# PRiME-project/PRiMEStereoMatch

Measured on AMD Instinct MI355X. Metric: cost-volume voxels/s (CVC+CVF+WTA), higher is better.
Workload: dtype f32; 1 GPU; synthetic 1920x1080 pair, D=256, float32 (BASELINE configs[3]); W=1920, H=1080, D=256, parallelism=1 GPU, kernel_variant=0, lr_check_on_gpu=False, batch=1, ranks=1, same_device=False, frames_in_flight=1

## Files before the change

include/primesm_hip.h:

```cpp
#ifndef PRIMESM_HIP_H
#define PRIMESM_HIP_H

#include <stddef.h>
#include <stdint.h>

#ifdef __cplusplus
extern "C" {
#endif

#define PSM_ABI_VERSION 1

typedef struct psm_ctx psm_ctx;

enum { PSM_F32 = 0, PSM_U8 = 1 };
enum { PSM_IMG_U8 = 0, PSM_IMG_F32 = 1 };
enum { PSM_LEFT = 0, PSM_RIGHT = 1 };
enum { PSM_STAGE_CVC = 0, PSM_STAGE_CVF = 1, PSM_STAGE_DISPSEL = 2, PSM_STAGE_PP = 3,
       PSM_STAGE_COUNT = 4 };
enum { PSM_K_PREP = 0, PSM_K_CVC = 1, PSM_K_GUIDE = 2, PSM_K_CVF_A = 3, PSM_K_CVF_B = 4,
       PSM_K_WTA = 5, PSM_K_MERGE = 6, PSM_K_BOX = 7, PSM_K_LRC = 8, PSM_K_CVF_F = 9, PSM_K_FGF = 10, PSM_K_WMF = 11,
       PSM_K_JWMF = 12, PSM_K_COUNT = 13 };
enum {
    PSM_OPT_ASYNC = 0,
    PSM_OPT_KERNEL_VARIANT = 1,
    PSM_OPT_PROFILE = 2,
    PSM_OPT_SEG_ROWS = 3,
    PSM_OPT_WAVES = 4,
    PSM_OPT_FLAGS = 5,
    PSM_OPT_GRAPH = 6,
    PSM_OPT_GATHER_STAGED = 7,
    PSM_OPT_FRAMES_IN_FLIGHT = 8
};

enum psm_flag {
    PSM_FLAG_MATERIALISE_COSTS = 128,
    PSM_FLAG_FGF_STORE = 4096,
    PSM_FLAG_STORE_FILTERED = 8192,
    PSM_FLAG_TWO_PHASE_ON = 1048576,
    PSM_FLAG_TWO_PHASE_OFF = 2097152,
    PSM_FLAG_WMF_DATAFLOW = 4194304,
    PSM_FLAG_WMF_TWO_SWEEPS = 8388608,
    PSM_FLAG_WMF_NO_CACHE = 16777216,
    PSM_FLAG_F32_TOL = 33554432,
    PSM_FLAG_FMA_SOLVE = 67108864,
    PSM_FLAGS_ALL = 128 | 4096 | 8192 | 1048576 | 2097152 | 4194304 | 8388608 | 16777216 | 33554432 | 67108864
};

int psm_device_count(void);

int psm_create(psm_ctx **out, int width, int height, int max_disp, int dtype, int device);

int psm_create_shard(psm_ctx **out, int width, int height, int max_disp, int d_begin, int d_end,
                     int dtype, int device);
int psm_create_shard_strided(psm_ctx **out, int width, int height, int max_disp, int d_first, int d_step,
                             int dtype, int device);

void psm_destroy(psm_ctx *ctx);

const char *psm_last_error(const psm_ctx *ctx);

int psm_set_option(psm_ctx *ctx, int option, int value);
int psm_set_stream(psm_ctx *ctx, void *hip_stream);
int psm_synchronize(psm_ctx *ctx);
int psm_release_scratch(psm_ctx *ctx);

int psm_upload_pair(psm_ctx *ctx, const void *l, const void *r, int channels, size_t stride_bytes,
                    int depth);

int psm_cost_construct(psm_ctx *ctx);

int psm_cost_filter(psm_ctx *ctx);

int psm_cost_filter_side(psm_ctx *ctx, int side);

int psm_cost_filter_fgf(psm_ctx *ctx, int subsample_rate);

int psm_disp_select(psm_ctx *ctx, uint8_t *lmap, uint8_t *rmap, size_t stride);

int psm_disp_select_partial(psm_ctx *ctx, void *dev_keys);
int psm_disp_select_partial_side(psm_ctx *ctx, int side, void *dev_keys_side);
int psm_set_key_buffer(psm_ctx *ctx, void *dev_keys);
int psm_partial_keys(psm_ctx *ctx, void **dev_keys, size_t *bytes);
int psm_disp_merge(psm_ctx *ctx, const void *dev_keys_all, int nranks, uint8_t *lmap,
                   uint8_t *rmap, size_t stride);
// ... 108 lines not shown
```

primestereomatch_amd/capi.py:

```python
from __future__ import annotations

import ctypes as C
import os

_HERE = os.path.dirname(os.path.abspath(__file__))
LIB_PATH = os.path.join(_HERE, "lib", "libprimesm_hip.so")

PSM_F32, PSM_U8 = 0, 1
PSM_IMG_U8, PSM_IMG_F32 = 0, 1
PSM_LEFT, PSM_RIGHT = 0, 1
PSM_STAGE_CVC, PSM_STAGE_CVF, PSM_STAGE_DISPSEL, PSM_STAGE_PP = 0, 1, 2, 3
(PSM_K_PREP, PSM_K_CVC, PSM_K_GUIDE, PSM_K_CVF_A, PSM_K_CVF_B, PSM_K_WTA, PSM_K_MERGE, PSM_K_BOX,
 PSM_K_LRC, PSM_K_CVF_F, PSM_K_FGF, PSM_K_WMF, PSM_K_JWMF) = range(13)
(PSM_OPT_ASYNC, PSM_OPT_KERNEL_VARIANT, PSM_OPT_PROFILE, PSM_OPT_SEG_ROWS, PSM_OPT_WAVES, PSM_OPT_FLAGS, PSM_OPT_GRAPH,
 PSM_OPT_GATHER_STAGED, PSM_OPT_FRAMES_IN_FLIGHT) = range(9)
PSM_FLAG_MATERIALISE_COSTS, PSM_FLAG_FGF_STORE, PSM_FLAG_STORE_FILTERED = 128, 4096, 8192
PSM_FLAG_TWO_PHASE_ON, PSM_FLAG_TWO_PHASE_OFF = 1048576, 2097152
PSM_FLAG_WMF_DATAFLOW, PSM_FLAG_WMF_TWO_SWEEPS, PSM_FLAG_WMF_NO_CACHE = 4194304, 8388608, 16777216
PSM_FLAG_F32_TOL = 33554432
PSM_FLAG_FMA_SOLVE = 67108864
PSM_SCORE_GIF, PSM_SCORE_SGM, PSM_SCORE_SGM_INT = 0, 1, 2
PSM_MASK_NONE, PSM_MASK_NONOCC, PSM_MASK_DISC = 0, 1, 2
PSM_SCORE_FLAT = 1


class Score(C.Structure):
    _fields_ = [("min_val", C.c_int32), ("max_val", C.c_int32), ("pixels", C.c_uint32), ("bad", C.c_uint32),
                ("err_sum", C.c_uint64), ("unit", C.c_int32), ("flags", C.c_uint32)]

    def as_dict(self):
        d = {name: int(getattr(self, name)) for name, _ in self._fields_}
        d["bp_percent"] = 100.0 * d["bad"] / d["pixels"]
        d["avg_err"] = (d["err_sum"] / d["pixels"]) / d["unit"] if d["unit"] else 0.0
        return d


_vp, _i, _sz = C.c_void_p, C.c_int, C.c_size_t
_pi, _pd = C.POINTER(C.c_int), C.POINTER(C.c_double)
SYMBOLS = [
    ("psm_device_count", _i, []),
    ("psm_create", _i, [C.POINTER(_vp), _i, _i, _i, _i, _i]),
    ("psm_create_shard", _i, [C.POINTER(_vp), _i, _i, _i, _i, _i, _i, _i]),
    ("psm_create_shard_strided", _i, [C.POINTER(_vp), _i, _i, _i, _i, _i, _i, _i]),
    ("psm_destroy", None, [_vp]),
    ("psm_last_error", C.c_char_p, [_vp]),
    ("psm_set_option", _i, [_vp, _i, _i]),
    ("psm_set_stream", _i, [_vp, _vp]),
    ("psm_synchronize", _i, [_vp]),
    ("psm_release_scratch", _i, [_vp]),
    ("psm_upload_pair", _i, [_vp, _vp, _vp, _i, _sz, _i]),
    ("psm_upload_pair_async", _i, [_vp, _vp, _vp, _i, _sz, _i]),
    ("psm_cost_construct", _i, [_vp]),
    ("psm_cost_filter", _i, [_vp]),
    ("psm_cost_filter_side", _i, [_vp, _i]),
    ("psm_cost_filter_fgf", _i, [_vp, _i]),
    ("psm_disp_select", _i, [_vp, _vp, _vp, _sz]),
    ("psm_disp_select_partial_side", _i, [_vp, _i, _vp]),
    ("psm_disp_select_partial", _i, [_vp, _vp]),
    ("psm_set_key_buffer", _i, [_vp, _vp]),
    ("psm_partial_keys", _i, [_vp, C.POINTER(_vp), C.POINTER(_sz)]),
    ("psm_disp_merge", _i, [_vp, _vp, _i, _vp, _vp, _sz]),
    ("psm_disp_merge_ctx", _i, [_vp, C.POINTER(_vp), _i, _vp, _vp, _sz]),
    ("psm_compute_batch", _i, [C.POINTER(_vp), _i]),
    ("psm_share_streams", _i, [C.POINTER(_vp), _i]),
    ("psm_download_maps", _i, [_vp, _vp, _vp, _sz]),
    ("psm_download_maps_async", _i, [_vp]),
    ("psm_download_maps_wait", _i, [_vp, _vp, _vp, _sz]),
    ("psm_lr_check", _i, [_vp, _vp, _vp, _sz]),
# ... 96 lines not shown
```

primestereomatch_amd/csrc/psm_api_core.cpp:

```cpp
#include "psm_ctx.h"

#include <chrono>
#include <cstdarg>
#include <cstdio>
#include <cstring>

using namespace psm;

namespace {
std::string g_create_error;
}

namespace psm {

double now_us()
{
    using namespace std::chrono;
    return duration_cast<duration<double, std::micro>>(steady_clock::now().time_since_epoch()).count();
}

int fail(psm_ctx *c, const char *fmt, ...)
{
    char buf[512];
    va_list ap;
// ... 296 lines not shown
    delete ctx;
}

const char *psm_last_error(const psm_ctx *ctx) { return ctx ? ctx->err.c_str() : g_create_error.c_str(); }

int psm_get_info(const psm_ctx *c, int *width, int *height, int *max_disp, int *d_begin, int *d_end, int *dtype, int *device)
{
    if (!c) return 1;
    if (width) *width = c->W;
    if (height) *height = c->H;
    if (max_disp) *max_disp = c->D;
    if (d_begin) *d_begin = c->d0;
    if (d_end) *d_end = c->d1;
    if (dtype) *dtype = c->dtype;
    if (device) *device = c->device;
    return 0;
}

int psm_set_option(psm_ctx *c, int option, int value)
{
    if (!c) return 1;
    switch (option) {
    case PSM_OPT_ASYNC: c->opt_async = value != 0; return 0;
    case PSM_OPT_KERNEL_VARIANT:
        if (value != 0 && value != 1) return fail(c, "psm_set_option: kernel variant %d unknown", value);
        c->opt_variant = value; return 0;
    case PSM_OPT_PROFILE:
        if (value < 0 || value > 2) return fail(c, "psm_set_option: profile mode %d not in {0,1,2}", value);
        c->opt_profile = value; return 0;
    case PSM_OPT_SEG_ROWS:
        if (value < 0) return fail(c, "psm_set_option: seg_rows %d < 0", value);
        c->march.seg_rows = value; return 0;
    case PSM_OPT_WAVES:
        if (value != 1 && value != 2 && value != 4 && value != 8) return fail(c, "psm_set_option: waves %d not in {1,2,4,8}", value);
        c->march.waves = value; return 0;
    case PSM_OPT_FLAGS:
        if (value & ~PSM_FLAGS_ALL) return fail(c, "psm_set_option: unknown flag bits 0x%x", value & ~PSM_FLAGS_ALL);
        if (c->dtype == PSM_U8) value &= ~(PSM_FLAG_FMA_SOLVE | PSM_FLAG_F32_TOL);
        if ((value & PSM_FLAG_F32_TOL) && (value & PSM_FLAG_FMA_SOLVE))
            return fail(c, "psm_set_option: PSM_FLAG_F32_TOL and PSM_FLAG_FMA_SOLVE exclude each other (one arithmetic variant at a time)");
        if ((value ^ c->march.flags) & PSM_FLAG_FMA_SOLVE) c->guid_rows = Rows{};
        c->march.flags = value; return 0;
    case PSM_OPT_GRAPH:
#ifdef PSM_EXPERIMENTS
        c->opt_graph = value != 0; return 0;
#else
        if (value != 0) return fail(c, "psm_set_option: PSM_OPT_GRAPH is not part of the product library (hipGraph replay of a batch measured slower than its plain launches)");
        return 0;
#endif
    case PSM_OPT_GATHER_STAGED: c->opt_gather_staged = value != 0; return 0;
    case PSM_OPT_FRAMES_IN_FLIGHT:
        if (value < 1 || value > 64) return fail(c, "psm_set_option: frames in flight %d not in [1, 64]", value);
        c->march.inflight = value; return 0;
    default: return fail(c, "psm_set_option: unknown option %d", option);
    }
}

int psm_set_stream(psm_ctx *c, void *hip_stream)
{
    if (!c) return 1;
    if (bind(c)) return 1;
    if (c->shared) return fail(c, "psm_set_stream: the context shares its streams with a batch (psm_share_streams)");
    PSM_HIP(c, hipStreamSynchronize(c->stream));
    c->stream = hip_stream ? (hipStream_t)hip_stream : c->own_stream;
    return 0;
}

int psm_synchronize(psm_ctx *c)
{
    if (!c) return 1;
    if (bind(c)) return 1;
    PSM_HIP(c, hipStreamSynchronize(c->stream));
    if (c->copy_stream) PSM_HIP(c, hipStreamSynchronize(c->copy_stream));
    if (c->down_stream && c->down_stream != c->copy_stream) PSM_HIP(c, hipStreamSynchronize(c->down_stream));
    return 0;
}

int psm_release_scratch(psm_ctx *c)
{
    if (!c) return 1;
    if (psm_synchronize(c)) return 1;
    (void)hipFree(c->wm_wts); c->wm_wts = nullptr; c->wm_wts_n = 0;
    (void)hipFree(c->wm_par); c->wm_par = nullptr;
    (void)hipFree(c->wm); c->wm = nullptr;
    (void)hipFree(c->gf_scratch); c->gf_scratch = nullptr; c->gf_scratch_bytes = 0;
    (void)hipFree(c->gather); c->gather = nullptr; c->gather_ranks = 0;
    (void)hipFree(c->fvol); c->fvol = nullptr;
    rectify_free(c, false);
    sgm_free(c);
    score_free(c, false);
    for (int k = 0; k < 2; ++k)
        if (c->xfer_pin[k]) { (void)hipHostFree(c->xfer_pin[k]); c->xfer_pin[k] = nullptr; c->xfer_pin_bytes[k] = 0; }
    (void)hipGetLastError();
    return 0;
}

int psm_share_streams(psm_ctx *const *ctxs, int n)
{
    if (!ctxs || n < 1 || !ctxs[0]) return fail(nullptr, "psm_share_streams: bad arguments");
    psm_ctx *c0 = ctxs[0];
    for (int i = 0; i < n; ++i) {
        if (!ctxs[i] || ctxs[i]->device != c0->device) return fail(c0, "psm_share_streams: context %d is NULL or on another device", i);
        if (ctxs[i]->shared) return fail(c0, "psm_share_streams: context %d already shares streams", i);
        for (int j = 0; j < i; ++j)
            if (ctxs[j] == ctxs[i]) return fail(c0, "psm_share_streams: context %d appears twice", i);
        if (ctxs[i]->stream != ctxs[i]->own_stream) return fail(c0, "psm_share_streams: context %d runs on a caller's stream (psm_set_stream)", i);
// ... 238 lines not shown
```

primestereomatch_amd/csrc/psm_kernels.h:

```cpp
#pragma once
#include <hip/hip_runtime.h>
#include <stdint.h>
#include "psm_live.h"

namespace psm {

struct Guidance {
    float4 *g1;
    float4 *g2;
    float4 *g3;
    float2 *g4;
};

struct March {
    int seg_rows;
    int waves;
    int flags;
    int dstep = 1;
    int inflight = 1;
    int ybeg = 0, yend = 0;
    int y0(int H) const { (void)H; return yend > ybeg ? ybeg : 0; }
    int y1(int H) const { return yend > ybeg ? yend : H; }
    int rows(int H) const { return y1(H) - y0(H); }
};

struct PcPair {
    const void *raw[2];
    Guidance g[2];
    uint8_t *p4[2];
    void *scratch;
    long long *keys;
    uint8_t *maps;
};
struct PcPairs {
    const PcPair *tab;
    int n;
    PcPair one;
};
void launch_prep_batch(hipStream_t s, const PcPair *tab, int npairs, size_t pitch, int depth_f32, int W, int H, bool u8_planes);
void launch_merge_batch(hipStream_t s, const PcPair *tab, int npairs, int W, int H);

void launch_copy_bytes(hipStream_t s, void *dst, const void *src, size_t bytes);
void launch_range_f32(hipStream_t s, const float *p, size_t n, unsigned *out);
void launch_prep(hipStream_t s, const void *src, size_t pitch, int depth_f32, int W, int H, float4 *g1, const void *src1 = nullptr,
                 float4 *g11 = nullptr);
void launch_guidance(hipStream_t s, const PcPairs &P, int W, int H, int ybeg, int yend, bool fma, int src = 0, size_t pitch = 0);
void launch_cvc(hipStream_t s, const float4 *g1_base, const float4 *g1_other, float *vol, int W, int H,
                int d_begin, int Dloc, int right, int ybeg, int yend);
void launch_cvf_a(hipStream_t s, int variant, March m, const float *vol, float4 *ab, Guidance g, int W,
                  int H, int Dloc, int ybeg, int yend);
void launch_cvf_b_direct(hipStream_t s, const float4 *ab, float *vol, Guidance g, int W, int H, int Dloc);
void launch_cvf_fused(hipStream_t s, March m, const float *vin, float *vout, Guidance g, int W, int H, int Dloc,
                      int ybeg, int yend, const float4 *g1_other, int d_begin, int cvc_mode, unsigned long long *ts = nullptr);
struct PcDev { int nxcd = 0, cus_per_xcd = 0; };
PcDev pc_dev();
enum { PC_STORE = 0, PC_PLANES = 1, PC_KEYS = 2, PC_BOTH = 4 };
struct PcPlan {
    int ngroups, nsegs, seg_rows, DC, nchunks, nbmax, nxcd;
    int cols;
    bool narrow;
    size_t rec_per_chunk;
    int rec_bytes;
    size_t scratch_bytes() const { return rec_per_chunk * (size_t)nchunks * rec_bytes; }
};
PcPlan pc_plan(int W, int rows, int Dloc, int seg_rows_opt, int form, int batch = 1, int inflight = 1);
PcPlan pc_plan_select(March m, int W, int H, int Dloc, int form, int npairs, bool batch);
int pc_seed_stride(int W, int rows, bool u8);
constexpr int PC_TS_SLOTS = 4096;
void launch_cvf_select(hipStream_t s, March m, const float *vin, Guidance g, int W, int H, int Dloc, const float4 *g1_other,
                       int d_begin, int cvc_mode, void *scratch, unsigned long long *ts = nullptr, const uint8_t *p4_own = nullptr,
                       const uint8_t *p4_other = nullptr);
void launch_chunk_min(hipStream_t s, March m, int W, int H, int Dloc, void *scratch, long long *keys, uint8_t *map);
void launch_cvf_select2(hipStream_t s, March m, const PcPairs &P, bool u8, int W, int H, int Dloc, int d_begin, unsigned long long *ts,
                        int sel, int step);
void launch_chunk_min2sides(hipStream_t s, March m, const PcPairs &P, int W, int H, int Dloc, bool to_maps, int d_begin, int sel, int step);
void launch_cvf_select_keys2(hipStream_t s, March m, const PcPairs &P, bool u8, int W, int H, int Dloc, int d_begin,
                             unsigned long long *ts, int sel, int step);
void launch_box8(hipStream_t s, int variant, March m, const float *vol, float *out, int W, int H, int Dloc);
void launch_wta(hipStream_t s, const float *vol, int W, int H, int d_begin, int Dloc, long long *keys,
                uint8_t *map);
void launch_merge(hipStream_t s, const long long *keys_all, size_t rank_stride, int nranks, int n,
                  uint8_t *map);
void launch_lr_check(hipStream_t s, const uint8_t *l, const uint8_t *r, int W, int H, uint8_t *lv,
                     uint8_t *rv);

void launch_fill_inv(hipStream_t s, uint8_t *dis, const uint8_t *valid, size_t side, int W, int H);

void launch_wgt_median(hipStream_t s, uint8_t *dis, const uint8_t *valid, const float4 *g1, int W, int H, int maxDis, int right,
                       int *nxt, int *prog, int *err);
constexpr int WM_LANE_MIN = 8192;
constexpr int WM_WROW = 20;
constexpr int WM_WPIX = 19 * WM_WROW;
struct WmSide {
    uint8_t *cur;
    const uint8_t *valid;
    const float4 *g1;
    uint8_t *orig, *newv, *chgb, *rowany;
    int *stamp, *list[2], *chg, *slot_of, *inv, *cnt;
    const float *wts;
};
struct WmPair { WmSide s[2]; };
void launch_wm_seed(hipStream_t s, const WmPair &p, int W, int H);
void launch_wm_sweep(hipStream_t s, const WmPair &p, int W, int H, int maxDis, int sw, bool cached, bool tail);
void launch_wm_weights(hipStream_t s, const float4 *g1, int W, int H, int right, const int *inv, const int *n_inv, int n, float *wts, int *slot_of);

void launch_fgf_setup(hipStream_t s, const float4 *g1, int W, int H, int sub, float4 *ism, float4 *msm, float4 *v1, float2 *v2);
void launch_fgf_model(hipStream_t s, const float *vol, const float4 *g1, const float4 *g1_other, int W, int H, int Dloc, int d_begin,
                      int sub, int cvc_mode, const float4 *msm, const float4 *v1, const float2 *v2, float4 *ab, float4 *mab);
void launch_fgf_apply(hipStream_t s, float *vol, const float4 *g1, int W, int H, int Dloc, int sub, const float4 *mab);
bool fgf_can_fuse_wta(int W);
void launch_fgf_apply_wta(hipStream_t s, const float4 *g1, int W, int H, int Dloc, int d_begin, int sub, const float4 *mab,
                          long long *keys);

// ... 151 lines not shown
```

primestereomatch_amd/csrc/psm_pc.hip:

```cpp
#include "psm_kernels.h"
#include "psm_cost.h"
#include "psm_dev.h"
#include "psm_live.h"
#include "../../include/primesm_hip.h"

#include <mutex>
#include <type_traits>

#include "psm_pc_debug.inc"

namespace psm {

typedef float f4v __attribute__((ext_vector_type(4)));

constexpr int PC_RING = 4;

template <int MODE, bool NARROW = false> struct PcLayout;
template <> struct PcLayout<0, false> { static constexpr int NA = 2, NB = 2, OUT_A = 52, OUT_B = 48, COLS = 96; };
template <> struct PcLayout<1, false> { static constexpr int NA = 2, NB = 2, OUT_A = 57, OUT_B = 54, COLS = 107; };
template <> struct PcLayout<2, false> : PcLayout<1, false> {};
template <> struct PcLayout<1, true> { static constexpr int NA = 1, NB = 1, OUT_A = 57, OUT_B = 50, COLS = 50; };
template <> struct PcLayout<2, true> : PcLayout<1, true> {};
constexpr int PC_K_LD_AUX = 0;
constexpr int PC_KEY_LD_AUX = 1;
// ... 4 lines not shown
{
    return __builtin_amdgcn_make_buffer_rsrc(const_cast<void *>(p), 0, bytes, 0x00020000);
}
__device__ __forceinline__ float pc_load1(__amdgpu_buffer_rsrc_t r, int voff, int soff)
{
    return __uint_as_float(__builtin_amdgcn_raw_buffer_load_b32(r, voff, soff, 0));
}
__device__ __forceinline__ float pc_load1_l2(__amdgpu_buffer_rsrc_t r, int voff, int soff)
{
    return __uint_as_float(__builtin_amdgcn_raw_buffer_load_b32(r, voff, soff, 16));
}
__device__ __forceinline__ float2 pc_load2(__amdgpu_buffer_rsrc_t r, int voff, int soff)
{
    const pc_u2 v = __builtin_amdgcn_raw_buffer_load_b64(r, voff, soff, 0);
    return make_float2(__uint_as_float(v.x), __uint_as_float(v.y));
}
__device__ __forceinline__ float4 pc_load4(__amdgpu_buffer_rsrc_t r, int voff, int soff)
{
    const pc_u4 v = __builtin_amdgcn_raw_buffer_load_b128(r, voff, soff, 0);
    return make_float4(__uint_as_float(v.x), __uint_as_float(v.y), __uint_as_float(v.z), __uint_as_float(v.w));
}

typedef unsigned pc_u3 __attribute__((ext_vector_type(3)));
__device__ __forceinline__ float3 pc_load3(__amdgpu_buffer_rsrc_t r, int voff, int soff)
{
    const pc_u3 v = __builtin_amdgcn_raw_buffer_load_b96(r, voff, soff, 0);
    return make_float3(__uint_as_float(v.x), __uint_as_float(v.y), __uint_as_float(v.z));
}

struct PcSide {
    const float4 *G1, *G2, *G3;
    const float2 *G4;
    const float4 *Gother;
    float *kcost;
    unsigned *kdisp;
};

constexpr int PC_LIVE_MAX = 6;
struct PcLive {
    int on;
    int lo, full;
    int pre[2], nshort[2], tot[2];
    int cnt[2][PC_LIVE_MAX];
};
__host__ __device__ __forceinline__ int pc_live_count(const PcLive &lv, int side, int g)
{
    const int k = g - (side ? lv.pre[1] : lv.pre[0]), ns = side ? lv.nshort[1] : lv.nshort[0];
    int c = lv.full;
#pragma unroll
    for (int i = 0; i < PC_LIVE_MAX; ++i)
        if (i == k && i < ns) c = side ? lv.cnt[1][i] : lv.cnt[0][i];
    return c;
}
struct PcSel {
    int sel, step;
    int nxcd;
    int spread;
    unsigned long long rec_total;
    int dstep;
    PcLive live;
};
__device__ __forceinline__ int pc_spread(const PcSel &o, int n, int i)
{
    if (o.spread > 1) {
        int r = 0, base = 0;
        for (; r < o.spread; ++r) {
            const int cnt = (n - r + o.spread - 1) / o.spread;
            if (i < base + cnt) break;
            base += cnt;
        }
        i = (i - base) * o.spread + r;
    }
    return i;
}

template <bool VEC4, int CVC, int MODE, bool U8 = false, bool BATCH = false, int VAR = 0, bool NARROW = false>
__global__ __launch_bounds__(64 * (PcLayout<MODE, NARROW>::NA + PcLayout<MODE, NARROW>::NB))
__attribute__((amdgpu_waves_per_eu(MODE == 2 ? 4 : 1, MODE == 2 ? 4 : 8)))
void k_cvf_pc(
    const float *__restrict__ vin, float *__restrict__ vout, const float4 *__restrict__ G1a, const float4 *__restrict__ G2a,
    const float4 *__restrict__ G3a, const float2 *__restrict__ G4a, int W, int H, int Dloc, int ngroups, int nsegs, int seg_rows,
    int ybeg, int yend, const float4 *__restrict__ Gothera, int d_begin, int DC, float *__restrict__ kcosta, unsigned *__restrict__ kdispa, int nbmax,
    PcSide side1, PcSel dyn, unsigned long long *__restrict__ ts, const PcPair *__restrict__ batch)
{
    constexpr bool TOL = VAR == 1, FMA = VAR == 2;
    static_assert(VAR >= 0 && VAR <= 2 && !(TOL && (U8 || MODE == 0)) && !(FMA && (U8 || BATCH)), "tolerance form: float select forms; FMA solve: float mode, single pair");
    if constexpr (BATCH) {
        static_assert(CVC == 3 && MODE != 0, "batched launches: both volumes per launch, select forms");
        const PcPair pp = batch[blockIdx.z];
        G1a = pp.g[0].g1; G2a = pp.g[0].g2; G3a = pp.g[0].g3; G4a = pp.g[0].g4; Gothera = pp.g[1].g1;
        side1.G1 = pp.g[1].g1; side1.G2 = pp.g[1].g2; side1.G3 = pp.g[1].g3; side1.G4 = pp.g[1].g4; side1.Gother = pp.g[0].g1;
        if (U8) { vin = (const float *)pp.p4[0]; vout = (float *)pp.p4[1]; }
        if (MODE == 1) {
            kcosta = (float *)pp.scratch;
            kdispa = (unsigned *)(kcosta + 4 * dyn.rec_total);
            side1.kcost = (float *)((char *)pp.scratch + dyn.rec_total * 20);
            side1.kdisp = (unsigned *)(side1.kcost + 4 * dyn.rec_total);
        } else {
            kcosta = (float *)pp.keys;
            side1.kcost = (float *)(pp.keys + (size_t)W * H);
        }
    }
    const bool right = CVC == 2 || (CVC == 3 && blockIdx.y == 1);
    const bool s1 = CVC == 3 && blockIdx.y == 1;
    const float4 *const G1 = s1 ? side1.G1 : G1a, *const G2 = s1 ? side1.G2 : G2a, *const G3 = s1 ? side1.G3 : G3a;
    const float2 *const G4 = s1 ? side1.G4 : G4a;
    const float4 *const Gother = s1 ? side1.Gother : Gothera;
    float *const kcost = s1 ? side1.kcost : kcosta;
    unsigned *const kdisp = s1 ? side1.kdisp : kdispa;
    static_assert(!NARROW || (MODE != 0 && CVC == 3), "the narrow layout exists for the two-volume select forms");
    using L = PcLayout<MODE, NARROW>;
    constexpr int PC_NA = L::NA, PC_NB = L::NB, PC_OUT_A = L::OUT_A, PC_OUT_B = L::OUT_B, PC_COLS = L::COLS;
    constexpr int PC_MCOLS = PC_NA * PC_OUT_A;
    constexpr bool SCALED = MODE != 0;
    constexpr float QSCALE = SCALED ? 0x1p-12f : 1.0f;
#define PSM_BOX(N) (SCALED ? (float)(N) : box_out(N))
    static_assert(PC_MCOLS >= PC_COLS + 7 && PC_OUT_A <= 57 && PC_OUT_B <= 57 && (MODE != 0 || (PC_COLS % 4) == 0), "bad producer/consumer layout");
    __shared__ __attribute__((aligned(16))) float4 ring[PC_RING][4][PC_MCOLS];
    __shared__ __attribute__((aligned(16))) float qbuf[MODE == 0 ? 2 : 1][MODE == 0 ? 4 : 1][MODE == 0 ? PC_COLS : 4];
    int id = blockIdx.x;
    const int npairs = ngroups * nsegs;
    const PcLive &lv = dyn.live;
    const int ltot = s1 ? lv.tot[1] : lv.tot[0];
    const int nitems = nsegs * ltot;
    const int ipx = (nitems + dyn.nxcd - 1) / dyn.nxcd;
    const int xcd = id % dyn.nxcd, jj = id / dyn.nxcd;
    const int item = xcd * ipx + jj;
    if (jj >= ipx || item >= nitems) return;
    if (ts != nullptr && threadIdx.x == 0) {
        (void)__hip_atomic_fetch_min(ts, (unsigned long long)wall_clock64(), __ATOMIC_RELAXED, __HIP_MEMORY_SCOPE_AGENT);
        if (blockIdx.x == 0 && blockIdx.y == 0) ts[2 * PC_TS_SLOTS] = (unsigned long long)MODE;
    }
    const int seg = item / ltot;
    int g, gi = item - seg * ltot, gn = lv.full;
    {
        const int pre = s1 ? lv.pre[1] : lv.pre[0], ns = s1 ? lv.nshort[1] : lv.nshort[0];
        if (gi < pre * lv.full) { g = gi / lv.full; gi -= g * lv.full; }
        else {
            gi -= pre * lv.full;
            g = pre;
            bool found = false;
#pragma unroll
            for (int k = 0; k < PC_LIVE_MAX; ++k) {
                const int c = s1 ? lv.cnt[1][k] : lv.cnt[0][k];
                if (!found && k < ns) {
                    if (gi < c) { found = true; gn = c; }
                    else { gi -= c; ++g; }
                }
            }
            if (!found) { const int q = gi / lv.full; g += q; gi -= q * lv.full; }
        }
    }
    const int pair = seg * ngroups + g;
    const int ch = lv.lo + gi;
    const int sl0 = pc_sel_index(dyn.sel, dyn.step, MODE == 2 ? lv.lo + pc_spread(dyn, gn, gi) : ch);
    const int wave = __builtin_amdgcn_readfirstlane(threadIdx.x >> 6), lane = threadIdx.x & 63;
    const bool is_a = wave < PC_NA;
    const int xg = g * PC_COLS;
    const int xm0 = xg - 4;
    const int y0 = ybeg + seg * seg_rows, y1 = min(yend, y0 + seg_rows);
    const int mstart = max(0, y0 - 4);
    const int mend = min(H - 1, max(y1 + 2, 4 - y0));
    const int nbA = (mend - mstart + 1 + 3) >> 2;
    const int nf = (y1 - y0) + 7;
    const int nbB = (nf + 3) >> 2;
    const int iters = nbB + 3;
    const int i1 = ((lane + 1) & 63) << 2, i2 = ((lane + 2) & 63) << 2, i4 = ((lane + 4) & 63) << 2;
    (void)i1;
    const size_t HW = (size_t)H * W;

    PC_TRACE_BEGIN()
    int ds_lo = 0, ds_hi = MODE == 1 ? min(DC, Dloc - ch * DC) : 1;
    if (MODE == 1 && lv.on) {
        const PcOwn own = {1, d_begin, dyn.dstep, dyn.sel, dyn.step};
        while (ds_lo < ds_hi && pc_dead_at(own, right, xg, xg + PC_COLS - 1, W, ch * DC + ds_lo)) ++ds_lo;
        while (ds_hi > ds_lo && pc_dead_at(own, right, xg, xg + PC_COLS - 1, W, ch * DC + ds_hi - 1)) --ds_hi;
        if (ds_lo >= ds_hi) return;
    }
    bool first = true;
    int rb = 0;
    for (int ds = ds_lo; ds < ds_hi; ++ds) {
    const int sl = MODE == 1 ? pc_sel_index(dyn.sel, dyn.step, ch * DC + ds) : sl0;
    const bool last_slice = ds == ds_hi - 1;
    if (is_a) {
        const int xa0 = xm0 + wave * PC_OUT_A;
        const int ci = r101c(xa0 - 4 + lane, W);
        const int xa = xa0 + lane;
        const int xac = xa < 0 ? 0 : (xa > W - 1 ? W - 1 : xa);
        const bool mvalid = lane < PC_OUT_A;
        const float *vd = vin + (size_t)sl * HW;
        const int dg = d_begin + dyn.dstep * sl;
        const bool inb = right ? (ci < W - dg) : (ci >= dg);
        const int cpart = right ? min(ci + dg, W - 1) : max(ci - dg, 0);
        const bool any_border = CVC != 0 && __builtin_amdgcn_ballot_w64(!inb) != 0;
        VTree t0 = {}, t1 = {}, t2 = {}, t3 = {};
        float pin[2];
        float4 oth[2], gin[2], o2[2], o3[2];
        float2 o4[2];
        constexpr bool LEANA = MODE == 2;
        const __amdgpu_buffer_rsrc_t rG1 = pc_rsrc(G1, (unsigned)HW * 16u), rG2 = pc_rsrc(G2, (unsigned)HW * 16u);
        const __amdgpu_buffer_rsrc_t rG3 = pc_rsrc(G3, (unsigned)HW * 16u), rG4 = pc_rsrc(G4, (unsigned)HW * 8u);
        const __amdgpu_buffer_rsrc_t rGo = pc_rsrc(CVC == 0 ? G1 : Gother, (unsigned)HW * 16u);
        const __amdgpu_buffer_rsrc_t rV = pc_rsrc(CVC == 0 ? (const void *)vd : (const void *)G1, (unsigned)HW * 4u);
        const __amdgpu_buffer_rsrc_t rPo = pc_rsrc(U8 ? (s1 ? (const void *)vin : (const void *)vout) : (const void *)G1, (unsigned)HW * 4u);
        unsigned po[2];
        const int vci = ci * 16, vcp = cpart * 16, vxa = xac * 16;
        constexpr bool DEEP = !LEANA;
#define PSM_ISSUE_PIX(SLOT, STEP)                                                       \
    {                                                                                   \
        const int row_ = r101c(mstart - 5 + (STEP), H) * W;                             \
        if (CVC == 0) pin[SLOT] = pc_load1(rV, vci >> 2, row_ * 4);                     \
        else if (U8) {            \
            po[SLOT] = __builtin_amdgcn_raw_buffer_load_b32(rPo, vcp >> 2, row_ * 4, 0); \
// ... 383 lines not shown
    const PcDev dev = pc_dev();
    PcPlan pl;
    pl.nxcd = dev.nxcd;
    constexpr int WIDE = PcLayout<1>::COLS, NARROW = PcLayout<1, true>::COLS;
    const bool select2 = (form & 3) != PC_STORE && (form & PC_BOTH);
    const int narrow_knob = PSM_KNOB("PSM_PC_NARROW", 0);
    pl.narrow = select2 && (narrow_knob ? narrow_knob == 1 : 2 * ((W + NARROW - 1) / NARROW) < 4 * ((W + WIDE - 1) / WIDE));
    const int cols = (form & 3) == PC_STORE ? PcLayout<0>::COLS : (pl.narrow ? NARROW : WIDE);
    pl.cols = cols;
    pl.ngroups = (W + cols - 1) / cols;
    const int kdiv = PSM_KNOB("PSM_PC_KDIV", rows < 128 ? 32 : 64);
    const int kmax = rows / kdiv > 1 ? rows / kdiv : 1;
    int dcs[5] = {1, 2, 4, 8, 16};
    int ndc = planes ? 5 : 1;
    if (planes && PSM_KNOB("PSM_PC_DC", 0) > 0) { dcs[0] = PSM_KNOB("PSM_PC_DC", 0); ndc = 1; }
    const long slots = PSM_KNOB("PSM_PC_SLOTS", (long)dev.cus_per_xcd * (keys ? 4 : 3) * (pl.narrow ? 2 : 1));
    const int conc = inflight > 1 ? inflight : 1;
    const int model_knob = PSM_KNOB("PSM_PC_MODEL", 0);
    const bool flow = model_knob ? model_knob == 1 : (sides * conc > 2 && (long)W * rows < 524288);
    auto cost_of = [&](int dc, int kk) -> long {
        const int nch = (Dloc + dc - 1) / dc;
        if (flow) {
            const double items = (double)sides * conc * pl.ngroups * kk * nch, len = dc * ((rows + kk - 1) / kk + 14) + 10.0;
            double c = items * len / ((double)slots * dev.nxcd) + 0.5 * len;
            if (planes && dc == 1) c *= 1.06;
            return (long)(c * 16.0);
        }
        const long per_xcd = ((long)sides * pl.ngroups * kk * nch + dev.nxcd - 1) / dev.nxcd;
        if (keys) {
            return (2 * ((per_xcd + slots - 1) / slots) + 3) * ((rows + kk - 1) / kk + 30) / 2;
        }
        const long rounds2 = 2 * ((per_xcd + slots - 1) / slots) + 1;
        long c = rounds2 * dc * ((rows + kk - 1) / kk + 14) / 2 + (planes ? 2L * sides * nch : 0);
        if (planes && dc == 1) c += (long)(0.06 * c * ((double)W * rows >= 2097152.0 ? 1.0 : (double)W * rows / 2097152.0));
        return c;
    };
    auto allowed = [&](int dc, int kk) { return (dc == dcs[0] || dc <= Dloc) && (seg_rows_opt <= 0 || kk == (rows + seg_rows_opt - 1) / seg_rows_opt); };
    long best = -1;
    for (int di = 0; di < ndc; ++di)
        for (int kk = 1; kk <= kmax && kk <= 32; ++kk)
            if (allowed(dcs[di], kk)) { const long c = cost_of(dcs[di], kk); if (best < 0 || c < best) best = c; }
    int bk = seg_rows_opt > 0 ? (rows + seg_rows_opt - 1) / seg_rows_opt : 1, bdc = dcs[0];
    for (int di = 0; di < ndc && best >= 0; ++di)
        for (int kk = 1; kk <= kmax && kk <= 32; ++kk)
            if (allowed(dcs[di], kk) && cost_of(dcs[di], kk) == best) { bk = kk; bdc = dcs[di]; di = ndc; break; }
    pl.seg_rows = seg_rows_opt > 0 ? seg_rows_opt : (rows + bk - 1) / bk;
    if (pl.seg_rows > rows) pl.seg_rows = rows;
    pl.nsegs = (rows + pl.seg_rows - 1) / pl.seg_rows;
    pl.DC = bdc;
    pl.nchunks = (Dloc + bdc - 1) / bdc;
    pl.nbmax = (pl.seg_rows + 7 + 3) / 4;
    pl.rec_per_chunk = (size_t)pl.ngroups * pl.nsegs * pl.nbmax * pl.cols;
    pl.rec_bytes = 20;
    return pl;
}

constexpr int PC_KEY_SPREAD = 4;

int pc_seed_stride(int W, int rows, bool u8)
{
    const int e = PSM_KNOB("PSM_PC_S", 0);
    if (e > 1) return e;
    if (rows < 200 || (u8 && (size_t)W * rows >= 1500000)) return 5;
    return 8;
}

static int pc_blocks(const PcPlan &pl, const PcLive &lv)
{
    const int items = pl.nsegs * (lv.tot[0] > lv.tot[1] ? lv.tot[0] : lv.tot[1]);
    return pl.nxcd * ((items + pl.nxcd - 1) / pl.nxcd);
}

struct PcArgs {
    const float *vin;
    float *vout;
    int W, H, Dloc, ybeg, yend, d_begin;
    PcSide side[2];
    PcSel sel;
    unsigned long long *ts;
    const PcPair *batch;
};

struct PcForm {
    int mode, cvc;
    bool u8;
    int var;
    bool batch, narrow, vec4;
};

template <int V> using pc_int = std::integral_constant<int, V>;
template <int... Vs, class Fn> static void pc_pick(int v, Fn &&fn) { (void)((v == Vs && (fn(pc_int<Vs>{}), true)) || ...); }
template <class Fn> static void pc_pick_bool(bool b, Fn &&fn) { if (b) fn(std::true_type{}); else fn(std::false_type{}); }

static void pc_launch(hipStream_t s, const PcPlan &pl, dim3 grid, const PcArgs &a, const PcForm &f)
{
    using F = std::false_type;
    using T = std::true_type;
    const bool planes = f.mode == PC_PLANES;
    const PcSide &s0 = a.side[0];
    if (grid.x == 0) return;
    auto go = [&](auto V4, auto CV, auto MD, auto U, auto BT, auto VR, auto NW) {
        using L = PcLayout<MD, NW>;
        hipLaunchKernelGGL(HIP_KERNEL_NAME(k_cvf_pc<V4, CV, MD, U, BT, VR, NW>), grid, dim3(64 * (L::NA + L::NB)), 0, s, a.vin, a.vout,
                           s0.G1, s0.G2, s0.G3, s0.G4, a.W, a.H, a.Dloc, pl.ngroups, pl.nsegs, pl.seg_rows, a.ybeg, a.yend, s0.Gother,
                           a.d_begin, planes ? pl.DC : 1, s0.kcost, s0.kdisp, planes ? pl.nbmax : 0, a.side[1], a.sel, a.ts, a.batch);
    };
// ... 57 lines not shown
    const PcLive lv = pc_live(W, pl.cols, pl.ngroups, Dloc, pl.DC, true, PcOwn{});
    PcArgs a = {u8 ? (const float *)p4_own : vin, u8 ? (float *)const_cast<uint8_t *>(p4_other) : nullptr, W, H, Dloc, m.y0(H), m.y1(H),
                d_begin, {}, PcSel{0, 1, pl.nxcd, 0, 0, 1, lv}, ts, nullptr};
    const PcSide k = pc_planes(pl, scratch, 0);
    a.side[0] = PcSide{gd.g1, gd.g2, gd.g3, gd.g4, g1_other, k.kcost, k.kdisp};
    pc_launch(s, pl, dim3(pc_blocks(pl, lv)), a, {PC_PLANES, cvc, u8, (m.flags & PSM_FLAG_FMA_SOLVE) ? 2 : 0, false, false, false});
}

void launch_chunk_min(hipStream_t s, March m, int W, int H, int Dloc, void *scratch, long long *keys, uint8_t *map)
{
    const PcPlan pl = pc_plan(W, m.rows(H), Dloc, m.seg_rows, PC_PLANES);
    pc_chunk_min(s, m, pl, W, H, 1, 1, scratch, keys, map, pc_live(W, pl.cols, pl.ngroups, Dloc, pl.DC, true, PcOwn{}));
}

static PcOwn pc_own(March m, int d_begin, int sel, int step) { return PcOwn{1, d_begin, m.dstep, sel, step}; }
PcPlan pc_plan_select(March m, int W, int H, int Dloc, int form, int npairs, bool batch)
{
    return pc_plan(W, m.rows(H), Dloc, m.seg_rows, form | PC_BOTH, npairs, batch ? 1 : m.inflight);
}

static PcArgs pc_args2(March m, const PcPlan &pl, int form, const PcPairs &P, bool u8, int W, int H, int Dloc, int d_begin, PcSel sel,
                       unsigned long long *ts)
{
    PcArgs a = {nullptr, nullptr, W, H, Dloc, m.y0(H), m.y1(H), d_begin, {}, sel, ts, P.tab};
    if (P.tab) return a;
    const PcPair &p = P.one;
    if (u8) { a.vin = (const float *)p.p4[0]; a.vout = (float *)p.p4[1]; }
    for (int v = 0; v < 2; ++v) {
        const PcSide k = form == PC_PLANES ? pc_planes(pl, p.scratch, v) : PcSide{};
        a.side[v] = PcSide{p.g[v].g1, p.g[v].g2, p.g[v].g3, p.g[v].g4, p.g[v ^ 1].g1, k.kcost, k.kdisp};
        if (form == PC_KEYS) a.side[v].kcost = (float *)(p.keys + v * (size_t)W * H);
    }
    return a;
}

void launch_cvf_select2(hipStream_t s, March m, const PcPairs &P, bool u8, int W, int H, int Dloc, int d_begin, unsigned long long *ts,
                        int sel, int step)
{
    const PcPlan pl = pc_plan_select(m, W, H, Dloc, PC_PLANES, P.n, P.tab != nullptr);
    const PcLive lv = pc_live(W, pl.cols, pl.ngroups, Dloc, pl.DC, true, pc_own(m, d_begin, sel, step));
    const unsigned long long rec_total = P.tab ? (unsigned long long)pl.rec_per_chunk * pl.nchunks : 0;
    const PcArgs a = pc_args2(m, pl, PC_PLANES, P, u8, W, H, Dloc, d_begin, PcSel{sel, step, pl.nxcd, 0, rec_total, m.dstep, lv}, ts);
    pc_launch(s, pl, dim3(pc_blocks(pl, lv), 2, P.n), a, {PC_PLANES, 3, u8, pc_var(m, u8), P.tab != nullptr, pl.narrow, false});
}

void launch_chunk_min2sides(hipStream_t s, March m, const PcPairs &P, int W, int H, int Dloc, bool to_maps, int d_begin, int sel, int step)
{
    const PcPlan pl = pc_plan_select(m, W, H, Dloc, PC_PLANES, P.n, P.tab != nullptr);
    const PcLive lv = pc_live(W, pl.cols, pl.ngroups, Dloc, pl.DC, true, pc_own(m, d_begin, sel, step));
    if (P.tab) pc_chunk_min(s, m, pl, W, H, 2, P.n, nullptr, nullptr, nullptr, lv, P.tab, to_maps);
    else pc_chunk_min(s, m, pl, W, H, 2, 1, P.one.scratch, P.one.keys, to_maps ? P.one.maps : nullptr, lv);
}

void launch_cvf_select_keys2(hipStream_t s, March m, const PcPairs &P, bool u8, int W, int H, int Dloc, int d_begin,
                             unsigned long long *ts, int sel, int step)
{
    const PcPlan pl = pc_plan_select(m, W, H, Dloc, PC_KEYS, P.n, P.tab != nullptr);
    const PcLive lv = pc_live(W, pl.cols, pl.ngroups, Dloc, 1, false, pc_own(m, d_begin, sel, step));
    const PcArgs a = pc_args2(m, pl, PC_KEYS, P, u8, W, H, Dloc, d_begin,
                              PcSel{sel, step, pl.nxcd, PSM_KNOB("PSM_PC_SPREAD", PC_KEY_SPREAD), 0, m.dstep, lv}, ts);
    pc_launch(s, pl, dim3(pc_blocks(pl, lv), 2, P.n), a, {PC_KEYS, 3, u8, pc_var(m, u8), P.tab != nullptr, pl.narrow, false});
}

}

extern "C" int psm_debug_pc_dead(int right, int xfirst, int xlast, int W, int dg, int dprev)
{
    return psm::pc_dead(right, xfirst, xlast, W, dg, dprev) ? 1 : 0;
}

extern "C" int psm_debug_pc_items(int W, int rows, int nsl, int form, int d_begin, int dstep, int sel, int step, int *out)
{
    using namespace psm;
    if (!out || W < 1 || rows < 1 || nsl < 1 || dstep < 1 || form < PC_STORE || form > PC_KEYS) return 1;
    March m = {};
    m.dstep = dstep;
    m.yend = rows;
    PcOwn own = pc_own(m, d_begin, sel, step);
    if (form == PC_STORE) own.on = 0;
    const PcPlan pl = form == PC_STORE ? pc_plan(W, rows, nsl, 0, PC_STORE) : pc_plan_select(m, W, rows, nsl, form, 1, false);
    const bool chunks = form == PC_PLANES;
    const PcLive lv = pc_live(W, pl.cols, pl.ngroups, nsl, chunks ? pl.DC : 1, chunks, own);
    int slices[2] = {0, 0};
    for (int side = 0; side < 2; ++side)
        for (int g = 0; g < pl.ngroups; ++g)
            for (int j = 0; j < nsl; ++j)
                slices[side] += pc_dead_at(own, side, g * pl.cols, g * pl.cols + pl.cols - 1, W, j) ? 0 : 1;
    const int v[12] = {pl.ngroups, pl.nsegs, pl.DC, pl.cols, lv.tot[0], lv.tot[1], pl.ngroups * (chunks ? pl.nchunks : nsl),
                       slices[0], slices[1], pc_blocks(pl, lv), lv.lo, 0};
    for (int i = 0; i < 12; ++i) out[i] = v[i];
    return 0;
}

extern "C" int psm_debug_pc_group_items(int W, int rows, int nsl, int form, int d_begin, int dstep, int sel, int step, int side, int g,
                                        int *out)
{
    using namespace psm;
    if (!out || W < 1 || rows < 1 || nsl < 1 || dstep < 1 || form < PC_PLANES || form > PC_KEYS || side < 0 || side > 1 || g < 0) return 1;
    March m = {};
    m.dstep = dstep;
    m.yend = rows;
    const PcPlan pl = pc_plan_select(m, W, rows, nsl, form, 1, false);
    if (g >= pl.ngroups) return 1;
    const bool chunks = form == PC_PLANES;
    const PcLive lv = pc_live(W, pl.cols, pl.ngroups, nsl, chunks ? pl.DC : 1, chunks, pc_own(m, d_begin, sel, step));
    out[0] = lv.lo;
    out[1] = pc_live_count(lv, side, g);
    return 0;
}
```

Baseline: 166.1 billion voxels/s.

## Split key-selection work into tall full-height and short segmented items

Adds an optional split of the key-selection launch into full-height (tall) items and row-segmented short items, controlled by a per-mille option or environment knob. Block-to-item mapping moves to a balanced per-XCD partition computed in a shared host/device helper. With default settings the tall share is zero, so the work decomposition matches the previous segmentation, with slightly different index arithmetic. The aim is to trade redundant halo rows against load balance across compute dies.

```diff
diff --git a/include/primesm_hip.h b/include/primesm_hip.h
--- a/include/primesm_hip.h
+++ b/include/primesm_hip.h
@@ -29,7 +29,8 @@
     PSM_OPT_FLAGS = 5,
     PSM_OPT_GRAPH = 6,
     PSM_OPT_GATHER_STAGED = 7,
-    PSM_OPT_FRAMES_IN_FLIGHT = 8
+    PSM_OPT_FRAMES_IN_FLIGHT = 8,
+    PSM_OPT_KEY_TALL = 9
 };
 
 enum psm_flag {
diff --git a/primestereomatch_amd/capi.py b/primestereomatch_amd/capi.py
--- a/primestereomatch_amd/capi.py
+++ b/primestereomatch_amd/capi.py
@@ -13,7 +13,7 @@
 (PSM_K_PREP, PSM_K_CVC, PSM_K_GUIDE, PSM_K_CVF_A, PSM_K_CVF_B, PSM_K_WTA, PSM_K_MERGE, PSM_K_BOX,
  PSM_K_LRC, PSM_K_CVF_F, PSM_K_FGF, PSM_K_WMF, PSM_K_JWMF) = range(13)
 (PSM_OPT_ASYNC, PSM_OPT_KERNEL_VARIANT, PSM_OPT_PROFILE, PSM_OPT_SEG_ROWS, PSM_OPT_WAVES, PSM_OPT_FLAGS, PSM_OPT_GRAPH,
- PSM_OPT_GATHER_STAGED, PSM_OPT_FRAMES_IN_FLIGHT) = range(9)
+ PSM_OPT_GATHER_STAGED, PSM_OPT_FRAMES_IN_FLIGHT, PSM_OPT_KEY_TALL) = range(10)
 PSM_FLAG_MATERIALISE_COSTS, PSM_FLAG_FGF_STORE, PSM_FLAG_STORE_FILTERED = 128, 4096, 8192
 PSM_FLAG_TWO_PHASE_ON, PSM_FLAG_TWO_PHASE_OFF = 1048576, 2097152
 PSM_FLAG_WMF_DATAFLOW, PSM_FLAG_WMF_TWO_SWEEPS, PSM_FLAG_WMF_NO_CACHE = 4194304, 8388608, 16777216
diff --git a/primestereomatch_amd/csrc/psm_api_core.cpp b/primestereomatch_amd/csrc/psm_api_core.cpp
--- a/primestereomatch_amd/csrc/psm_api_core.cpp
+++ b/primestereomatch_amd/csrc/psm_api_core.cpp
@@ -372,6 +372,9 @@
     case PSM_OPT_FRAMES_IN_FLIGHT:
         if (value < 1 || value > 64) return fail(c, "psm_set_option: frames in flight %d not in [1, 64]", value);
         c->march.inflight = value; return 0;
+    case PSM_OPT_KEY_TALL:
+        if (value < -1 || value > 1000) return fail(c, "psm_set_option: key tall share %d not in [-1, 1000] per mille", value);
+        c->march.key_tall = value; return 0;
     default: return fail(c, "psm_set_option: unknown option %d", option);
     }
 }
diff --git a/primestereomatch_amd/csrc/psm_kernels.h b/primestereomatch_amd/csrc/psm_kernels.h
--- a/primestereomatch_amd/csrc/psm_kernels.h
+++ b/primestereomatch_amd/csrc/psm_kernels.h
@@ -18,6 +18,7 @@
     int flags;
     int dstep = 1;
     int inflight = 1;
+    int key_tall = -1;
     int ybeg = 0, yend = 0;
     int y0(int H) const { (void)H; return yend > ybeg ? ybeg : 0; }
     int y1(int H) const { return yend > ybeg ? yend : H; }
@@ -59,6 +60,7 @@
     int ngroups, nsegs, seg_rows, DC, nchunks, nbmax, nxcd;
     int cols;
     bool narrow;
+    int tall = 0, short_rows = 0;
     size_t rec_per_chunk;
     int rec_bytes;
     size_t scratch_bytes() const { return rec_per_chunk * (size_t)nchunks * rec_bytes; }
diff --git a/primestereomatch_amd/csrc/psm_pc.hip b/primestereomatch_amd/csrc/psm_pc.hip
--- a/primestereomatch_amd/csrc/psm_pc.hip
+++ b/primestereomatch_amd/csrc/psm_pc.hip
@@ -80,6 +80,58 @@
         if (i == k && i < ns) c = side ? lv.cnt[1][i] : lv.cnt[0][i];
     return c;
 }
+struct PcGroupItem { int g, gi, gn; };
+__host__ __device__ __forceinline__ PcGroupItem pc_live_item(const PcLive &lv, int side, int idx)
+{
+    int g, gi = idx, gn = lv.full;
+    const int pre = side ? lv.pre[1] : lv.pre[0], ns = side ? lv.nshort[1] : lv.nshort[0];
+    if (gi < pre * lv.full) { g = gi / lv.full; gi -= g * lv.full; }
+    else {
+        gi -= pre * lv.full;
+        g = pre;
+        bool found = false;
+#pragma unroll
+        for (int k = 0; k < PC_LIVE_MAX; ++k) {
+            const int c = side ? lv.cnt[1][k] : lv.cnt[0][k];
+            if (!found && k < ns) {
+                if (gi < c) { found = true; gn = c; }
+                else { gi -= c; ++g; }
+            }
+        }
+        if (!found) { const int q = gi / lv.full; g += q; gi -= q * lv.full; }
+    }
+    return PcGroupItem{g, gi, gn};
+}
+__host__ __device__ __forceinline__ int pc_part_count(int n, int permille, int part)
+{
+    const int t = (int)((long long)n * permille / 1000);
+    return part ? n - t : t;
+}
+inline PcLive pc_live_part(const PcLive &lv, int ngroups, int permille, int part)
+{
+    PcLive p = lv;
+    p.full = pc_part_count(lv.full, permille, part);
+    for (int side = 0; side < 2; ++side) {
+        p.tot[side] = 0;
+        for (int g = 0; g < ngroups; ++g) p.tot[side] += pc_part_count(pc_live_count(lv, side, g), permille, part);
+        for (int i = 0; i < PC_LIVE_MAX; ++i) p.cnt[side][i] = pc_part_count(lv.cnt[side][i], permille, part);
+    }
+    return p;
+}
+struct PcKeyCut {
+    PcLive tall, shrt;
+    int nsegs, seg_rows;
+};
+inline int pc_key_blocks(const PcKeyCut &kc, int nxcd)
+{
+    int m = 0;
+    for (int side = 0; side < 2; ++side) {
+        const int nt = kc.tall.tot[side], ns = kc.nsegs * kc.shrt.tot[side];
+        const int p = (nt + nxcd - 1) / nxcd + (ns + nxcd - 1) / nxcd;
+        m = p > m ? p : m;
+    }
+    return nxcd * m;
+}
 struct PcSel {
     int sel, step;
     int nxcd;
@@ -87,8 +139,9 @@
     unsigned long long rec_total;
     int dstep;
     PcLive live;
+    PcKeyCut key;
 };
-__device__ __forceinline__ int pc_spread(const PcSel &o, int n, int i)
+__host__ __device__ __forceinline__ int pc_spread(const PcSel &o, int n, int i)
 {
     if (o.spread > 1) {
         int r = 0, base = 0;
@@ -100,6 +153,40 @@
         i = (i - base) * o.spread + r;
     }
     return i;
+}
+
+struct PcKeyItem { int valid, part, seg, g, sl, y0, y1; };
+__host__ __device__ __forceinline__ PcKeyItem pc_key_block(const PcSel &o, int side, int id, int ybeg, int yend)
+{
+    const PcKeyCut &kc = o.key;
+    const int nxcd = o.nxcd;
+    PcKeyItem it = {};
+    int pos, n;
+    const int ttot = side ? kc.tall.tot[1] : kc.tall.tot[0], stot = side ? kc.shrt.tot[1] : kc.shrt.tot[0];
+    const int nt = ttot, ns = kc.nsegs * stot;
+    const int xcd = id % nxcd, jj = id / nxcd;
+    const int tq = nt / nxcd, tr = nt - tq * nxcd, tn = tq + (xcd < tr ? 1 : 0), t0 = xcd * tq + (xcd < tr ? xcd : tr);
+    const int sq = ns / nxcd, sr = ns - sq * nxcd, sn = sq + (xcd < sr ? 1 : 0), s0 = xcd * sq + (xcd < sr ? xcd : sr);
+    if (id < 0 || jj >= tn + sn) return it;
+    it.valid = 1;
+    if (jj < tn) {
+        const PcGroupItem gi = pc_live_item(kc.tall, side, t0 + jj);
+        it.g = gi.g; pos = gi.gi;
+        n = gi.gn + pc_live_count(kc.shrt, side, gi.g);
+        it.y0 = ybeg; it.y1 = yend;
+    } else {
+        const int idx = s0 + jj - tn;
+        it.part = 1;
+        it.seg = idx / stot;
+        const PcGroupItem gi = pc_live_item(kc.shrt, side, idx - it.seg * stot);
+        const int first = pc_live_count(kc.tall, side, gi.g);
+        it.g = gi.g; pos = first + gi.gi;
+        n = first + gi.gn;
+        it.y0 = ybeg + it.seg * kc.seg_rows;
+        it.y1 = it.y0 + kc.seg_rows < yend ? it.y0 + kc.seg_rows : yend;
+    }
+    it.sl = pc_sel_index(o.sel, o.step, o.live.lo + pc_spread(o, n, pos));
+    return it;
 }
 
 template <bool VEC4, int CVC, int MODE, bool U8 = false, bool BATCH = false, int VAR = 0, bool NARROW = false>
@@ -149,44 +236,35 @@
     int id = blockIdx.x;
     const int npairs = ngroups * nsegs;
     const PcLive &lv = dyn.live;
-    const int ltot = s1 ? lv.tot[1] : lv.tot[0];
-    const int nitems = nsegs * ltot;
-    const int ipx = (nitems + dyn.nxcd - 1) / dyn.nxcd;
-    const int xcd = id % dyn.nxcd, jj = id / dyn.nxcd;
-    const int item = xcd * ipx + jj;
-    if (jj >= ipx || item >= nitems) return;
+    int seg, g, gi = 0, gn = 0, y0, y1;
+    int slk = 0;
+    if constexpr (MODE == 2 && !BATCH) {
+        const PcKeyItem it = pc_key_block(dyn, s1 ? 1 : 0, id, ybeg, yend);
+        if (!it.valid) return;
+        seg = it.seg; g = it.g; slk = it.sl; y0 = it.y0; y1 = it.y1;
+    } else {
+        const int ltot = s1 ? lv.tot[1] : lv.tot[0];
+        const int nitems = nsegs * ltot;
+        const int ipx = (nitems + dyn.nxcd - 1) / dyn.nxcd;
+        const int xcd = id % dyn.nxcd, jj = id / dyn.nxcd;
+        const int item = xcd * ipx + jj;
+        if (jj >= ipx || item >= nitems) return;
+        seg = item / ltot;
+        const PcGroupItem it = pc_live_item(lv, s1 ? 1 : 0, item - seg * ltot);
+        g = it.g; gi = it.gi; gn = it.gn;
+        y0 = ybeg + seg * seg_rows; y1 = min(yend, y0 + seg_rows);
+    }
     if (ts != nullptr && threadIdx.x == 0) {
         (void)__hip_atomic_fetch_min(ts, (unsigned long long)wall_clock64(), __ATOMIC_RELAXED, __HIP_MEMORY_SCOPE_AGENT);
         if (blockIdx.x == 0 && blockIdx.y == 0) ts[2 * PC_TS_SLOTS] = (unsigned long long)MODE;
     }
-    const int seg = item / ltot;
-    int g, gi = item - seg * ltot, gn = lv.full;
-    {
-        const int pre = s1 ? lv.pre[1] : lv.pre[0], ns = s1 ? lv.nshort[1] : lv.nshort[0];
-        if (gi < pre * lv.full) { g = gi / lv.full; gi -= g * lv.full; }
-        else {
-            gi -= pre * lv.full;
-            g = pre;
-            bool found = false;
-#pragma unroll
-            for (int k = 0; k < PC_LIVE_MAX; ++k) {
-                const int c = s1 ? lv.cnt[1][k] : lv.cnt[0][k];
-                if (!found && k < ns) {
-                    if (gi < c) { found = true; gn = c; }
-                    else { gi -= c; ++g; }
-                }
-            }
-            if (!found) { const int q = gi / lv.full; g += q; gi -= q * lv.full; }
-        }
-    }
     const int pair = seg * ngroups + g;
     const int ch = lv.lo + gi;
-    const int sl0 = pc_sel_index(dyn.sel, dyn.step, MODE == 2 ? lv.lo + pc_spread(dyn, gn, gi) : ch);
+    const int sl0 = MODE == 2 && !BATCH ? slk : pc_sel_index(dyn.sel, dyn.step, MODE == 2 ? lv.lo + pc_spread(dyn, gn, gi) : ch);
     const int wave = __builtin_amdgcn_readfirstlane(threadIdx.x >> 6), lane = threadIdx.x & 63;
     const bool is_a = wave < PC_NA;
     const int xg = g * PC_COLS;
     const int xm0 = xg - 4;
-    const int y0 = ybeg + seg * seg_rows, y1 = min(yend, y0 + seg_rows);
     const int mstart = max(0, y0 - 4);
     const int mend = min(H - 1, max(y1 + 2, 4 - y0));
     const int nbA = (mend - mstart + 1 + 3) >> 2;
@@ -676,6 +754,13 @@
     pl.nbmax = (pl.seg_rows + 7 + 3) / 4;
     pl.rec_per_chunk = (size_t)pl.ngroups * pl.nsegs * pl.nbmax * pl.cols;
     pl.rec_bytes = 20;
+    pl.tall = 0;
+    pl.short_rows = pl.seg_rows;
+    if (keys && PSM_KNOB("PSM_PC_TALL", 0) > 0) {
+        pl.tall = PSM_KNOB("PSM_PC_TALL", 0) - 1;
+        pl.short_rows = PSM_KNOB("PSM_PC_SEGS", pl.seg_rows);
+    }
+    if (pl.short_rows > rows) pl.short_rows = rows;
     return pl;
 }
 
@@ -839,14 +924,30 @@
     else pc_chunk_min(s, m, pl, W, H, 2, 1, P.one.scratch, P.one.keys, to_maps ? P.one.maps : nullptr, lv);
 }
 
+static PcKeyCut pc_key_cut(March m, const PcPlan &pl, const PcLive &lv, bool u8, bool batch, int rows)
+{
+    const bool forced = m.key_tall >= 0 && !batch, planned = m.key_tall < 0 && !batch && !u8 && !(m.yend > m.ybeg) && pl.tall > 0;
+    const int tall = forced ? m.key_tall : (planned ? pl.tall : 0);
+    PcKeyCut kc;
+    kc.tall = pc_live_part(lv, pl.ngroups, tall, 0);
+    kc.shrt = pc_live_part(lv, pl.ngroups, tall, 1);
+    kc.seg_rows = tall > 0 && (planned || m.seg_rows <= 0) ? pl.short_rows : pl.seg_rows;
+    if (kc.seg_rows < 1) kc.seg_rows = 1;
+    if (kc.seg_rows > rows) kc.seg_rows = rows;
+    kc.nsegs = (rows + kc.seg_rows - 1) / kc.seg_rows;
+    return kc;
+}
+
 void launch_cvf_select_keys2(hipStream_t s, March m, const PcPairs &P, bool u8, int W, int H, int Dloc, int d_begin,
                              unsigned long long *ts, int sel, int step)
 {
     const PcPlan pl = pc_plan_select(m, W, H, Dloc, PC_KEYS, P.n, P.tab != nullptr);
     const PcLive lv = pc_live(W, pl.cols, pl.ngroups, Dloc, 1, false, pc_own(m, d_begin, sel, step));
+    const PcKeyCut kc = pc_key_cut(m, pl, lv, u8, P.tab != nullptr, m.rows(H));
     const PcArgs a = pc_args2(m, pl, PC_KEYS, P, u8, W, H, Dloc, d_begin,
-                              PcSel{sel, step, pl.nxcd, PSM_KNOB("PSM_PC_SPREAD", PC_KEY_SPREAD), 0, m.dstep, lv}, ts);
-    pc_launch(s, pl, dim3(pc_blocks(pl, lv), 2, P.n), a, {PC_KEYS, 3, u8, pc_var(m, u8), P.tab != nullptr, pl.narrow, false});
+                              PcSel{sel, step, pl.nxcd, PSM_KNOB("PSM_PC_SPREAD", PC_KEY_SPREAD), 0, m.dstep, lv, kc}, ts);
+    pc_launch(s, pl, dim3(P.tab ? pc_blocks(pl, lv) : pc_key_blocks(kc, pl.nxcd), 2, P.n), a,
+              {PC_KEYS, 3, u8, pc_var(m, u8), P.tab != nullptr, pl.narrow, false});
 }
 
 }
@@ -895,3 +996,39 @@
     out[1] = pc_live_count(lv, side, g);
     return 0;
 }
+
+extern "C" int psm_debug_pc_key_blocks(int W, int rows, int nsl, int d_begin, int dstep, int sel, int step, int tall_permille,
+                                       int seg_rows, int side, int first, int count, int *out)
+{
+    using namespace psm;
+    if (!out || W < 1 || rows < 1 || nsl < 1 || dstep < 1 || side < 0 || side > 1 || tall_permille < -1 || tall_permille > 1000 ||
+        seg_rows < 0 || first < -1 || count < 0)
+        return 1;
+    March m = {};
+    m.dstep = dstep;
+    m.yend = rows;
+    m.seg_rows = seg_rows;
+    m.key_tall = tall_permille;
+    const PcPlan pl = pc_plan_select(m, W, rows, nsl, PC_KEYS, 1, false);
+    const PcLive lv = pc_live(W, pl.cols, pl.ngroups, nsl, 1, false, pc_own(m, d_begin, sel, step));
+    m.yend = 0;
+    const PcKeyCut kc = pc_key_cut(m, pl, lv, false, false, rows);
+    const PcSel o = {sel, step, pl.nxcd, PC_KEY_SPREAD, 0, dstep, lv, kc};
+    if (first < 0) {
+        const int v[6] = {pc_key_blocks(kc, pl.nxcd), pl.nxcd, pl.ngroups, pl.cols, kc.nsegs, kc.seg_rows};
+        for (int i = 0; i < 6; ++i) out[i] = v[i];
+        return 0;
+    }
+    for (int i = 0; i < count; ++i) {
+        const PcKeyItem it = pc_key_block(o, side, first + i, 0, rows);
+        const int v[6] = {it.valid, it.part, it.g, it.sl, it.y0, it.y1};
+        for (int k = 0; k < 6; ++k) out[6 * i + k] = v[k];
+    }
+    return 0;
+}
+
+extern "C" int psm_debug_pc_key_block(int W, int rows, int nsl, int d_begin, int dstep, int sel, int step, int tall_permille,
+                                      int seg_rows, int side, int block, int out[6])
+{
+    return psm_debug_pc_key_blocks(W, rows, nsl, d_begin, dstep, sel, step, tall_permille, seg_rows, side, block, 1, out);
+}
```

Result: no change. 166.6 billion voxels/s (median of 6 runs) (+0.3%).
